# zhyever/Amodal-Depth-Anything

Measured on AMD Instinct MI355X. Metric: images/sec at 518x518 bs=32 ViT-L (AmodalDAv2 forward), higher is better.
Workload: dtype f16

## Files before the change

### amodal-depth-anything_amd/csrc/ada_igemm.hip

```cpp
#include <math.h>
#include <stdarg.h>
#include <stdlib.h>
#include <atomic>
#include <mutex>
#include <type_traits>
#include "ada_common.h"

namespace {


enum { EPI_STD = 0, EPI_GELU = 1, EPI_SHUFFLE = 2, EPI_SWIGLU = 3, EPI_TAIL = 4 };

#ifndef ADA_EPI_NT
#define ADA_EPI_NT 4
#endif
ADA_DEV float4 ld_res4(const float* ptr) {
#if ADA_EPI_NT & 1
    const f32x4 v = __builtin_nontemporal_load((const f32x4*)ptr);
    return make_float4(v[0], v[1], v[2], v[3]);
#else
    return *(const float4*)ptr;
#endif
}
ADA_DEV void st_f32x4(float* ptr, float4 v) {
#if ADA_EPI_NT & 2
    const f32x4 t = {v.x, v.y, v.z, v.w};
    __builtin_nontemporal_store(t, (f32x4*)ptr);
#else
    *(float4*)ptr = v;
#endif
}

struct IgemmDev {
    int M, N, K, a_mode;
// ... 12 lines not shown
    float* out_f32;
    long ldo_f32;
    int map_f32;
    op_t* out_op;
    long ldo_op;
    int map_op;
    int map_h, map_w;
    FastDiv dMapW, dMapHW;
    int shuffle_s, shuffle_c;
    int split_seg;
    int a_dup_seg;
    int split_f8;
    int f8_from, f8_mid;
    unsigned f8_scales;
    int bias_row_mod;
    FastDiv dBiasMod;
    int a_wrap;
    int tap_cols;
    unsigned long long tap_bits[3];
    FastDiv dShC, dShS;
    const float* tail_w;
    float tail_b;
    int tail_act;
    int tiles_m, tiles_n;
    int cps;
    int variant;
    int group_n;
    unsigned long long* dbg;
};

ADA_DEV float gelu_erf(float x) {
    const float a = __builtin_fminf(__builtin_fabsf(x), 12.0f);
    float q = -3.2904290173e-05f;
    q = __builtin_fmaf(q, a, 7.6214928455e-04f);
    q = __builtin_fmaf(q, a, -8.0387993652e-03f);
    q = __builtin_fmaf(q, a, 5.3315321524e-02f);
    q = __builtin_fmaf(q, a, 4.5887145819e-01f);
    q = __builtin_fmaf(q, a, 1.1511568259e+00f);
    q = __builtin_fmaf(q, a, 9.9999958888e-01f);
    const float tail = __builtin_amdgcn_exp2f(-q);
    return __builtin_fmaf(-a, tail, __builtin_fmaxf(x, 0.0f));
}

ADA_DEV void gelu_erf4(float4& v) {
    v.x = gelu_erf(v.x);
    v.y = gelu_erf(v.y);
// ... 477 lines not shown
            if (flags & ADA_EP_BIAS) bias4 = *(const float4*)(p.bias + n);
            tail4 = *(const float4*)(p.tail_w + n);
        }
#pragma unroll
        for (int i = 0; i < TI; ++i) {
            dump(i, 0);
#pragma unroll
            for (int k = 0; k < 32 / RPI; ++k) {
                const int row = k * RPI + rsub;
                const int m = mbase + i * 32 + row;
                const float4 v = *(const float4*)(slab + row * SW + 4 * cg);
                float part = __builtin_fmaxf(v.x + bias4.x, 0.f) * tail4.x + __builtin_fmaxf(v.y + bias4.y, 0.f) * tail4.y +
                             __builtin_fmaxf(v.z + bias4.z, 0.f) * tail4.z + __builtin_fmaxf(v.w + bias4.w, 0.f) * tail4.w;
#pragma unroll
                for (int o = 1; o < CG; o <<= 1) part += __shfl_xor(part, o);
                if (cg == 0 && m < p.M) {
                    float d = part + p.tail_b;
                    if (p.tail_act == ADA_ACT_SIGMOID) d = 1.0f / (1.0f + __expf(-d));
                    else if (p.tail_act == ADA_ACT_RELU) d = __builtin_fmaxf(d, 0.0f);
                    p.out_f32[m] = d;
                }
            }
        }
    } else if (EPI != EPI_SHUFFLE && m0 + BM <= p.M && n0 + BN <= p.N && p.res_row_mod == 0 && p.bias_row_mod == 0 &&
               (!p.out_op || p.map_op == ADA_MAP_PLAIN || (p.map_op == ADA_MAP_PAD && p.map_w >= 8)) &&
               (!p.out_f32 || p.map_f32 == ADA_MAP_PLAIN) &&
               (p.out_f32 || (flags & ADA_EP_RESIDUAL) || (p.ldo_op & 7) == 0)) {
        const bool has_bias = (flags & ADA_EP_BIAS) != 0, has_gamma = (flags & ADA_EP_GAMMA) != 0;
        if (!p.out_f32 && !(flags & ADA_EP_RESIDUAL)) {
            constexpr int CG = GW / 8, RPI = 64 / CG;
            const int rsub = lane / CG, cg = CG == 8 ? ((lane - (rsub >> 1)) & 7) : lane % CG;
            const bool relu = (flags & ADA_EP_RELU_OP) != 0;
            const long ld = p.ldo_op;
#pragma unroll
            for (int g = 0; g < NG; ++g) {
                const int n = nwave + g * GW + 8 * cg;
                float4 b0 = make_float4(0, 0, 0, 0), b1 = b0, g0 = make_float4(1, 1, 1, 1), g1 = g0;
                if (has_bias) { b0 = *(const float4*)(p.bias + n); b1 = *(const float4*)(p.bias + n + 4); }
                if (has_gamma) { g0 = *(const float4*)(p.gamma + n); g1 = *(const float4*)(p.gamma + n + 4); }
                op_t* dst = p.out_op + (long)(mbase + rsub) * ld + n;
                const bool pad = p.map_op == ADA_MAP_PAD;
#pragma unroll
                for (int i = 0; i < TI; ++i) {
                    dump(i, g);
                    PadWalk walk;
                    if (pad) walk = pad_start(p, (uint32_t)(mbase + i * 32 + rsub));
// ... 438 lines not shown
    ADA_REQUIRE(a->out_f32 || a->out_op, ADA_EINVAL, "ada_igemm: no output buffer");
    ADA_REQUIRE((long)a->M < (1L << 24), ADA_EUNSUPPORTED, "ada_igemm: M=%d exceeds 2^24 rows", a->M);
    ADA_REQUIRE(a->a_dup_seg >= 0 && a->a_dup_seg % 64 == 0, ADA_EINVAL, "ada_igemm: a_dup_seg=%d must be a non-negative multiple of 64", a->a_dup_seg);
    if (a->a_dup_seg > 0) {
        const long taps = a->a_mode == ADA_A_CONV3 ? 9 : 1;
        ADA_REQUIRE((long)a->K == 3L * taps * a->a_dup_seg && a->lda >= 2L * a->a_dup_seg, ADA_EINVAL,
                    "ada_igemm: a split A operand needs K == %ld * a_dup_seg and lda >= 2 * a_dup_seg (K=%d a_dup_seg=%d lda=%ld)", 3 * taps, a->K, a->a_dup_seg, (long)a->lda);
    }
    if (a->a_mode == ADA_A_CONV3) {
        ADA_REQUIRE(a->lda % 64 == 0, ADA_EINVAL, "ada_igemm: CONV3 needs lda %% 64 == 0 (got %ld)", (long)a->lda);
        ADA_REQUIRE(a->a_dup_seg > 0 || a->K == 9 * a->lda, ADA_EINVAL, "ada_igemm: CONV3 needs K == 9*lda (K=%d lda=%ld)", a->K, (long)a->lda);
        ADA_REQUIRE(a->Ho > 0 && a->Wo > 0 && (a->stride == 1 || a->stride == 2), ADA_EINVAL, "ada_igemm: bad conv geometry");
        ADA_REQUIRE(a->Hp >= (a->Ho - 1) * a->stride + 3 && a->Wp >= (a->Wo - 1) * a->stride + 3, ADA_EINVAL,
                    "ada_igemm: padded input %dx%d too small for output %dx%d stride %d", a->Hp, a->Wp, a->Ho, a->Wo, a->stride);
        ADA_REQUIRE(a->M % (a->Ho * a->Wo) == 0, ADA_EINVAL, "ada_igemm: M must be batch*Ho*Wo");
    } else {
        ADA_REQUIRE(a->a_mode == ADA_A_PLAIN, ADA_EINVAL, "ada_igemm: unknown a_mode %d", a->a_mode);
        ADA_REQUIRE(a->a_dup_seg > 0 || a->a_wrap > 0 || a->lda >= a->K, ADA_EINVAL, "ada_igemm: lda=%ld < K=%d", (long)a->lda, a->K);
    }
    const int f = a->flags;
    ADA_REQUIRE(!(f & ADA_EP_BIAS) || a->bias, ADA_EINVAL, "ada_igemm: EP_BIAS without bias");
    ADA_REQUIRE(!(f & ADA_EP_GAMMA) || a->gamma, ADA_EINVAL, "ada_igemm: EP_GAMMA without gamma");
    ADA_REQUIRE(!(f & ADA_EP_RESIDUAL) || a->res, ADA_EINVAL, "ada_igemm: EP_RESIDUAL without res");
    const bool tail = (f & ADA_EP_TAIL) != 0, swiglu = (f & ADA_EP_SWIGLU) != 0;
    const bool shuffle = a->out_op && a->map_op == ADA_MAP_SHUFFLE;
    ADA_REQUIRE(a->N % 4 == 0, ADA_EUNSUPPORTED, "ada_igemm: N=%d must be a multiple of 4", a->N);
    ADA_REQUIRE(!a->out_f32 || tail || (a->ldo_f32 % 4 == 0 && ((uintptr_t)a->out_f32 % 16) == 0), ADA_EINVAL, "ada_igemm: out_f32 must be 16-byte aligned with ldo %% 4 == 0");
    ADA_REQUIRE(!a->out_op || (a->ldo_op % 4 == 0 && ((uintptr_t)a->out_op % 8) == 0), ADA_EINVAL, "ada_igemm: out_op must be 8-byte aligned with ldo %% 4 == 0");
    ADA_REQUIRE(!(f & ADA_EP_RESIDUAL) || (a->ldr % 4 == 0 && ((uintptr_t)a->res % 16) == 0), ADA_EINVAL, "ada_igemm: res must be 16-byte aligned with ldr %% 4 == 0");
    ADA_REQUIRE(!(f & ADA_EP_BIAS) || ((uintptr_t)a->bias % 16) == 0, ADA_EINVAL, "ada_igemm: bias must be 16-byte aligned");
    ADA_REQUIRE(!(f & ADA_EP_GAMMA) || ((uintptr_t)a->gamma % 16) == 0, ADA_EINVAL, "ada_igemm: gamma must be 16-byte aligned");
    if (tail) {
        ADA_REQUIRE(a->tail_w && a->out_f32, ADA_EINVAL, "ada_igemm: EP_TAIL needs tail_w and out_f32");
        ADA_REQUIRE(((uintptr_t)a->tail_w % 16) == 0, ADA_EINVAL, "ada_igemm: tail_w must be 16-byte aligned");
        ADA_REQUIRE(a->N <= 64, ADA_EUNSUPPORTED, "ada_igemm: EP_TAIL supports N <= 64 (got %d)", a->N);
        ADA_REQUIRE(!swiglu && !shuffle && !(f & ADA_EP_GELU), ADA_EUNSUPPORTED, "ada_igemm: EP_TAIL cannot be combined with other epilogues");
    }
    if (swiglu) {
        ADA_REQUIRE(a->N % 64 == 0 && a->out_op && !a->out_f32, ADA_EINVAL, "ada_igemm: EP_SWIGLU needs N %% 64 == 0 and only out_op");
        ADA_REQUIRE(a->map_op == ADA_MAP_PLAIN && !(f & (ADA_EP_GELU | ADA_EP_GAMMA | ADA_EP_RESIDUAL)), ADA_EUNSUPPORTED,
                    "ada_igemm: EP_SWIGLU supports bias + MAP_PLAIN only");
    }
    const int maps_needing_grid = (a->out_op && (a->map_op == ADA_MAP_PAD || a->map_op == ADA_MAP_SHUFFLE));
    if (maps_needing_grid) {
        ADA_REQUIRE(a->map_h > 0 && a->map_w > 0 && a->M % (a->map_h * a->map_w) == 0, ADA_EINVAL, "ada_igemm: bad output grid %dx%d for M=%d", a->map_h, a->map_w, a->M);
    }
    if (shuffle) {
        ADA_REQUIRE(a->shuffle_s > 0 && a->shuffle_c > 0 && a->N == a->shuffle_s * a->shuffle_s * a->shuffle_c, ADA_EINVAL,
                    "ada_igemm: SHUFFLE needs N == s*s*c");
        ADA_REQUIRE(a->shuffle_c % 4 == 0 && !a->out_f32 && !(f & ADA_EP_GELU), ADA_EUNSUPPORTED, "ada_igemm: SHUFFLE needs c %% 4 == 0, operand output only");
    }
    const int split_abs = a->split_seg < 0 ? -a->split_seg : a->split_seg;
    if (a->split_seg != 0) {
        ADA_REQUIRE(a->out_op && split_abs % 8 == 0, ADA_EINVAL, "ada_igemm: split_seg needs out_op and a multiple of 8");
        ADA_REQUIRE(a->split_seg > 0 || !shuffle || (a->shuffle_c % 8 == 0 && !(f & ADA_EP_RESIDUAL) && a->ldo_op % 8 == 0), ADA_EUNSUPPORTED,
                    "ada_igemm: the fp8 form of a split output (split_seg < 0) behind MAP_SHUFFLE needs shuffle_c %% 8 == 0, ldo_op %% 8 == 0 and no residual");
        const int cols = shuffle ? a->shuffle_c : swiglu ? a->N / 2 : a->N;
        ADA_REQUIRE(cols <= split_abs && a->ldo_op >= 2L * split_abs, ADA_EINVAL, "ada_igemm: split_seg=%d too small for %d columns / ldo_op=%ld", a->split_seg, cols, (long)a->ldo_op);
    }
    if (a->bias_row_mod != 0) {
        ADA_REQUIRE(a->bias_row_mod > 0 && (f & ADA_EP_BIAS) && a->out_op && !a->out_f32 && !(f & ADA_EP_RESIDUAL) && !tail && !swiglu && !shuffle &&
                    a->ldo_op % 8 == 0 && a->N % 4 == 0, ADA_EUNSUPPORTED,
                    "ada_igemm: bias_row_mod (a bias vector per group of rows) is implemented for operand-typed outputs with ldo_op %% 8 == 0 (bias / GELU epilogues)");
    }
    if (a->a_wrap != 0) {
        ADA_REQUIRE(a->a_mode == ADA_A_PLAIN && a->a_dup_seg == 0 && a->a_wrap > 0 && a->a_wrap % 64 == 0 && a->K == 2 * a->a_wrap && a->lda >= a->a_wrap, ADA_EINVAL,
                    "ada_igemm: a_wrap=%d needs a plain operand, K == 2 * a_wrap (K=%d) and lda >= a_wrap", a->a_wrap, a->K);
    }
    if (a->f8_from != 0) {
        const long per = a->a_mode == ADA_A_CONV3 ? a->lda : (long)a->K;
        ADA_REQUIRE(a->a_dup_seg == 0 && a->a_wrap == 0, ADA_EINVAL, "ada_igemm: f8_from excludes a_dup_seg / a_wrap");
        ADA_REQUIRE(a->f8_from > 0 && a->f8_from % 64 == 0 && a->f8_mid % 64 == 0 && a->f8_from <= a->f8_mid && a->f8_mid <= per && a->f8_from < per, ADA_EINVAL,
                    "ada_igemm: f8_from=%d / f8_mid=%d must be multiples of 64 with 0 < f8_from <= f8_mid <= %ld (the period of the k-walk)", a->f8_from, a->f8_mid, per);
    }
    if (a->tap_cols != 0) {
        ADA_REQUIRE(a->a_mode == ADA_A_CONV3 && a->tap_cols > 0 && a->N % a->tap_cols == 0 && a->N / a->tap_cols <= 16, ADA_EINVAL,
                    "ada_igemm: tap_cols=%d needs a CONV3 operand and N = (1..16) * tap_cols (N=%d)", a->tap_cols, a->N);
        for (int i = 0; i < a->N / a->tap_cols; ++i)
            ADA_REQUIRE(a->tap_mask[i] != 0 && a->tap_mask[i] < 512, ADA_EINVAL, "ada_igemm: tap_mask[%d]=0x%x must name 1..9 of the taps", i, (unsigned)a->tap_mask[i]);
    }
// ... 14 lines not shown
    d.dResMod = make_fastdiv(a->res_row_mod > 0 ? a->res_row_mod : 1);
    d.flags = a->flags;
    d.out_f32 = a->out_f32; d.ldo_f32 = a->ldo_f32; d.map_f32 = a->map_f32;
    d.out_op = (op_t*)a->out_op; d.ldo_op = a->ldo_op; d.map_op = a->map_op;
    d.map_h = a->map_h; d.map_w = a->map_w;
    const bool token = (a->out_f32 && a->map_f32 == ADA_MAP_TOKEN) || (a->out_op && a->map_op == ADA_MAP_TOKEN);
    d.dMapW = make_fastdiv(a->map_w > 0 ? a->map_w : 1);
    d.dMapHW = make_fastdiv(token ? a->map_h : (a->map_h > 0 && a->map_w > 0 ? a->map_h * a->map_w : 1));
    d.shuffle_s = a->shuffle_s; d.shuffle_c = a->shuffle_c;
    d.split_seg = split_abs;
    d.split_f8 = a->split_seg < 0;
    d.f8_from = a->f8_from / 64; d.f8_mid = a->f8_mid / 64; d.f8_scales = a->f8_scales;
    d.a_dup_seg = a->a_dup_seg;
    d.a_wrap = a->a_wrap;
    d.bias_row_mod = a->bias_row_mod;
    d.dBiasMod = make_fastdiv(a->bias_row_mod > 0 ? a->bias_row_mod : 1);
    d.tap_cols = a->tap_cols;
    d.tap_bits[0] = d.tap_bits[1] = d.tap_bits[2] = 0;
    if (a->tap_cols > 0)
        for (int i = 0; i < a->N / a->tap_cols; ++i) d.tap_bits[i / 7] |= (unsigned long long)a->tap_mask[i] << (9 * (i % 7));
    d.dShC = make_fastdiv(a->shuffle_c > 0 ? a->shuffle_c : 1);
    d.dShS = make_fastdiv(a->shuffle_s > 0 ? a->shuffle_s : 1);
    d.tail_w = a->tail_w; d.tail_b = a->tail_b; d.tail_act = a->tail_act;
    d.cps = 0;
    d.group_n = 1;
    d.tiles_m = d.tiles_n = 0;

    apply_env_presets();
    const int force = g_force_tile.load(std::memory_order_relaxed);
    d.dbg = g_dbg.load(std::memory_order_relaxed);
    d.variant = g_variant.load(std::memory_order_relaxed);
    hipStream_t s = (hipStream_t)stream;
    if (tail) return launch_epi<EPI_TAIL>(d, s, a->N <= 32 ? 0 : 1);
    if (swiglu) return launch_epi<EPI_SWIGLU>(d, s, force);
    if (shuffle) return launch_epi<EPI_SHUFFLE>(d, s, force);
    if (f & ADA_EP_GELU) return launch_epi<EPI_GELU>(d, s, force);
    return launch_epi<EPI_STD>(d, s, force);
}
```

### amodal-depth-anything_amd/hip_ext/__init__.py

```python
from __future__ import annotations

import ctypes
import os
from ctypes import c_char_p, c_double, c_float, c_int, c_int32, c_int64, c_uint16, c_void_p
from typing import Optional

import torch

_HERE = os.path.dirname(os.path.abspath(__file__))
_CSRC = os.path.join(os.path.dirname(_HERE), "csrc")

ABI_VERSION = 8
DT_F32, DT_F16, DT_BF16 = 0, 1, 2
A_PLAIN, A_CONV3 = 0, 1
MAP_PLAIN, MAP_PAD, MAP_TOKEN, MAP_SHUFFLE = 0, 1, 2, 3
EP_BIAS, EP_GELU, EP_GAMMA, EP_RESIDUAL, EP_RELU_OP, EP_SWIGLU, EP_TAIL, EP_RELU_F32 = 0x1, 0x2, 0x4, 0x8, 0x10, 0x20, 0x40, 0x80
ACT_NONE, ACT_SIGMOID, ACT_RELU = 0, 1, 2

EXPORTS = (
    "ada_abi_version", "ada_operand_dtype", "ada_last_error", "ada_igemm", "ada_attention_fwd", "ada_attention_ex",
    "ada_pos_embed_resize", "ada_layernorm_fwd", "ada_layernorm_ex", "ada_patchify", "ada_write_cls", "ada_bilinear_fwd", "ada_selftest",
    "ada_minmax_fwd", "ada_depth_stats_fwd", "ada_token_diversity_fwd", "ada_normalize_fwd", "ada_blend_fwd", "ada_depth_eval_fwd", "ada_tile_blend_fwd", "ada_dpt_tail_fwd", "ada_tapsum_resize_fwd",
    "ada_debug_set_tile", "ada_debug_set_variant", "ada_debug_set_group", "ada_debug_last_tile",
    "ada_debug_set_timestamps", "ada_debug_set_attention_variant", "ada_debug_count_saturated",
)

EVAL_N, EVAL_SUM_P, EVAL_SUM_G, EVAL_SUM_PP, EVAL_SUM_PG, EVAL_ABS_REL, EVAL_SQ_REL, EVAL_SQ, EVAL_LOG_SQ, EVAL_LOG, \
    EVAL_LOG10_ABS, EVAL_D1, EVAL_D2, EVAL_D3, EVAL_INV_SQ = range(15)
EVAL_NSUM = 16


class IgemmArgs(ctypes.Structure):
    _fields_ = [
        ("M", c_int32), ("N", c_int32), ("K", c_int32), ("a_mode", c_int32),
        ("A", c_void_p), ("lda", c_int64),
        ("Ho", c_int32), ("Wo", c_int32), ("Hp", c_int32), ("Wp", c_int32), ("stride", c_int32),
        ("W", c_void_p), ("bias", c_void_p), ("gamma", c_void_p), ("res", c_void_p), ("ldr", c_int64),
        ("res_row_mod", c_int32), ("res_row_off", c_int32), ("flags", c_int32),
        ("out_f32", c_void_p), ("ldo_f32", c_int64), ("map_f32", c_int32),
        ("out_op", c_void_p), ("ldo_op", c_int64), ("map_op", c_int32),
        ("map_h", c_int32), ("map_w", c_int32), ("shuffle_s", c_int32), ("shuffle_c", c_int32),
        ("tail_w", c_void_p), ("tail_b", c_float), ("tail_act", c_int32),
        ("split_seg", c_int32), ("a_dup_seg", c_int32),
        ("tap_cols", c_int32), ("tap_mask", c_uint16 * 16), ("a_wrap", c_int32), ("bias_row_mod", c_int32),
        ("f8_from", c_int32), ("f8_mid", c_int32), ("f8_scales", ctypes.c_uint32),
    ]


class LayerNormArgs(ctypes.Structure):
    _fields_ = [
        ("in_", c_void_p), ("ld_in", c_int64), ("rows_out", c_int32), ("dim", c_int32), ("group_in", c_int32), ("skip", c_int32),
        ("weight", c_void_p), ("bias", c_void_p), ("eps", c_float),
        ("out_op", c_void_p), ("ld_op", c_int64), ("map_op", c_int32), ("map_h", c_int32), ("map_w", c_int32), ("relu", c_int32),
        ("out_f32", c_void_p), ("ld_f32", c_int64), ("split_seg", c_int32),
        ("weight2", c_void_p), ("bias2", c_void_p), ("out2_op", c_void_p), ("ld2_op", c_int64),
        ("out2_group", c_int32), ("out2_skip", c_int32), ("split_seg2", c_int32), ("unshuffle_s", c_int32), ("tap_bias", c_void_p), ("identity", c_int32),
    ]


class HipExtError(RuntimeError):
    pass


_lib = None
_lib_path = None


def library_path(bf16: bool = False) -> str:
# ... 119 lines not shown
        ev1.record(torch.cuda.current_stream())
        self.records.setdefault(name, []).append((ev0, ev1, float(work)))

    def summary(self):
        out = {}
        for name, recs in self.records.items():
            ms = sum(a.elapsed_time(b) for a, b, _ in recs)
            out[name] = dict(launches=len(recs), ms_total=ms, ms_avg=ms / len(recs), work_total=sum(w for _, _, w in recs))
        return out


_timer: Optional[KernelTimer] = None


def set_timer(t: Optional[KernelTimer]):
    global _timer
    _timer = t


def igemm(*, M, N, K, A, lda, W, k_alg=None, a_mode=A_PLAIN, conv=None, bias=None, gamma=None, res=None, ldr=0,
          res_row_mod=0, res_row_off=0, flags=0, out_f32=None, ldo_f32=0, map_f32=MAP_PLAIN, out_op=None, ldo_op=0,
          map_op=MAP_PLAIN, map_h=0, map_w=0, shuffle_s=0, shuffle_c=0, tail_w=None, tail_b=0.0, tail_act=ACT_NONE, split_seg=0,
          a_dup_seg=0, tap_cols=0, tap_mask=None, a_wrap=0, bias_row_mod=0,
          f8_from=0, f8_mid=0, f8_scales=0):
    op = operand_dtype()
    a = IgemmArgs()
    a.M, a.N, a.K, a.a_mode = M, N, K, a_mode
    a.A, a.lda = _dev(A, "A", op), lda
    if conv is not None:
        a.Ho, a.Wo, a.Hp, a.Wp, a.stride = conv
    a.W = _dev(W, "W", op)
    a.bias = _opt(bias, "bias", torch.float32)
    a.gamma = _opt(gamma, "gamma", torch.float32)
    a.res, a.ldr = _opt(res, "res", torch.float32), ldr
    a.res_row_mod, a.res_row_off, a.flags = res_row_mod, res_row_off, flags
    a.out_f32, a.ldo_f32, a.map_f32 = _opt(out_f32, "out_f32", torch.float32), ldo_f32, map_f32
    a.out_op, a.ldo_op, a.map_op = _opt(out_op, "out_op", op), ldo_op, map_op
    a.map_h, a.map_w, a.shuffle_s, a.shuffle_c = map_h, map_w, shuffle_s, shuffle_c
    a.tail_w, a.tail_b, a.tail_act = _opt(tail_w, "tail_w", torch.float32), tail_b, tail_act
    a.split_seg = split_seg
    a.a_dup_seg = a_dup_seg
    a.a_wrap = a_wrap
    a.bias_row_mod = bias_row_mod
    a.f8_from, a.f8_mid, a.f8_scales = f8_from, f8_mid, f8_scales
    if tap_cols:
        a.tap_cols = tap_cols
        for i, m in enumerate(tap_mask):
            a.tap_mask[i] = int(m)
    if _timer is not None and _timer.active:
        ev = _timer.start()
        _check(load().ada_igemm(ctypes.byref(a), _stream()), "ada_igemm")
        _timer.stop("igemm", ev, 2.0 * M * N * (k_alg if k_alg is not None else K))
    else:
        _check(load().ada_igemm(ctypes.byref(a), _stream()), "ada_igemm")
    if _tile_log is not None:
        _tile_log.append((M, N, K, load().ada_debug_last_tile()))


def attention(qkv: torch.Tensor, out: torch.Tensor, batch: int, n_tokens: int, heads: int, ld_out: int = 0, split_seg: int = 0):
    op = operand_dtype()
    ev = _timer.start() if (_timer is not None and _timer.active) else None
    if ld_out or split_seg:
        _check(load().ada_attention_ex(_dev(qkv, "qkv", op), _dev(out, "out", op), batch, n_tokens, heads, ld_out, split_seg, _stream()), "ada_attention_ex")
    else:
        _check(load().ada_attention_fwd(_dev(qkv, "qkv", op), _dev(out, "out", op), batch, n_tokens, heads, _stream()),
               "ada_attention_fwd")
    if ev is not None:
# ... 181 lines not shown
```

### amodal-depth-anything_amd/hip_ext/engine.py

```python
from __future__ import annotations

import math
import os
import threading
from collections import OrderedDict
from typing import Dict, Optional

import torch
import torch.nn.functional as F

from . import (A_CONV3, ACT_NONE, ACT_RELU, ACT_SIGMOID, EP_BIAS, EP_GAMMA, EP_GELU, EP_RELU_OP, EP_RESIDUAL,
               EP_SWIGLU, EP_TAIL, MAP_PAD, MAP_SHUFFLE, MAP_TOKEN, HipExtError)
from . import attention as k_attention
from . import bilinear as _bilinear
from . import count_saturated
from . import dpt_tail as k_dpt_tail
from . import igemm as _igemm
from . import layernorm as _layernorm
from . import debug_epoch, instrumented, operand_dtype
from . import depth_stats as k_depth_stats
from . import token_diversity as k_token_diversity
from . import patchify as k_patchify
from . import pos_embed_resize as k_pos_embed_resize
from . import tapsum_resize as k_tapsum_resize
from . import write_cls as k_write_cls

_probe = None


def _probed(kernel, launch):
    def run(*a, **kw):
        launch(*a, **kw)
        t = kw.get("out_op")
        if _probe is not None and t is not None and t.is_contiguous():
            c = torch.zeros(1, dtype=torch.int64, device=t.device)
            count_saturated(t, c)
            _probe.append((f"{kernel} #{len(_probe)} {list(t.shape)}", c))
    return run


k_igemm, k_layernorm, k_bilinear = _probed("igemm", _igemm), _probed("layernorm", _layernorm), _probed("bilinear", _bilinear)

PATCH = 14
LN_EPS = 1e-6
HEAD_GROUPS = ("proj", "projw", "rs0", "rs1", "rs3") + tuple(f"{f}{i}" for f in ("ip", "rn", "rcu", "out") for i in range(4)) + ("oc1", "oc2")
HEAD_ALIASES = {"tok": ("proj", "rs0", "rs1", "rs3"), "ip": tuple(f"ip{i}" for i in range(4)), "rn": tuple(f"rn{i}" for i in range(4)),
                "rcu": tuple(f"rcu{i}" for i in range(4)), "out": tuple(f"out{i}" for i in range(4))}
FUSED_TAIL = os.environ.get("ADA_FUSED_TAIL", "1") == "1"
SUBPIXEL = os.environ.get("ADA_SUBPIXEL", "1") == "1"
SUBPIXEL_SPLIT = os.environ.get("ADA_SUBPIXEL_SPLIT", "1") != "0"
OC1_COMMUTE_SPLIT = os.environ.get("ADA_OC1_COMMUTE_SPLIT", "1") != "0"
STAT_CHUNKS = 8
OC1_COMMUTE = os.environ.get("ADA_OC1_COMMUTE", "1") != "0"


_F8_ENV = os.environ.get("ADA_F8_CORR", "1")
F8_CORR = _F8_ENV != "0"
F8_ENC, F8_HEAD = _F8_ENV in ("1", "enc"), _F8_ENV in ("1", "head")
F8_A_SCALES = 117 | (127 << 16)


def f8_weight_split(wm: torch.Tensor, op, taps: int = 1):
    n = wm.shape[0]
    k = wm.shape[1] // taps
    assert wm.shape[1] == taps * k and k % 128 == 0, (wm.shape, taps)
    w = wm.reshape(n, taps, k).float()
    hi = w.to(op)
    lo = w - hi.float()

    def enc(t):
        m = float(t.abs().max())
        sh = max(-100, min(100, int(math.floor(math.log2(448.0 / m))))) if m > 0 else 0
        q = (t.float() * (2.0 ** sh)).clamp(-448.0, 448.0)
        try:
            b = q.to(torch.float8_e4m3fn).view(torch.uint8)
        except (RuntimeError, TypeError):
# ... 330 lines not shown
            self.o = z(T, wide * D)
            hidden = pw_.blocks[0]["hidden"]
            self.hd = z(T, wide * hidden)
        self.taps = [z(P, m * D) for _ in range(4)]
        G = (D + 63) // 64
        Gi = 0 if head_only else pw_.pe_seg // 64
        self.stat_buf = z(B * (STAT_CHUNKS + G + Gi) * 2, dtype=torch.float32)
        self.stat_sums = self.stat_buf[:B * STAT_CHUNKS * 2].view(B, STAT_CHUNKS, 2)
        self.stat_div = self.stat_buf[B * STAT_CHUNKS * 2:B * (STAT_CHUNKS + G) * 2].view(B, G, 2)
        self.stat_in = self.stat_buf[B * (STAT_CHUNKS + G) * 2:].view(B, Gi, 2) if Gi else None
        if pw_.readout:
            self.cls_op = [z(B, m * D) for _ in range(4)]
            self.cls_bias = [z(B, D, dtype=torch.float32) for _ in range(4)]
            self.taps_ro = [z(P, m * D) for _ in range(4)]
        self.grid = [(4 * ph, 4 * pw), (2 * ph, 2 * pw), (ph, pw), ((ph - 1) // 2 + 1, (pw - 1) // 2 + 1)]
        oc = pw_.oc
        ocp = [_r64(c) for c in oc]
        self.ocp, self.Fp = ocp, Fp
        self.tp = {i: z(B, ph + 2, pw + 2, (2 if pw_.sp[i].get("split") else 1) * ocp[i]) for i in pw_.sp}
        self.t0 = None if 0 in pw_.sp else z(P, mm("rs0") * ocp[0])
        self.t1 = None if 1 in pw_.sp else z(P, mm("rs1") * ocp[1])
        self.pre3 = z(B, ph + 2, pw + 2, mm("rs3") * ocp[3])
        self.L = [None if i in pw_.sp else z(B, g[0] + 2, g[1] + 2, mm(f"{first}{i}") * ocp[i]) for i, g in enumerate(self.grid)]
        if pw_.amodal_head:
            self.ipf = [z(B * g[0] * g[1], oc[i], dtype=torch.float32) for i, g in enumerate(self.grid)]
            self.L2 = [z(B, g[0] + 2, g[1] + 2, mm(f"rn{i}") * ocp[i]) for i, g in enumerate(self.grid)]
        self.rnx = [z(B * g[0] * g[1], Fch, dtype=torch.float32) for g in self.grid]
        self.spf = {} if pw_.amodal_head else {i: z(B * self.grid[i][0] * self.grid[i][1], Fch, dtype=torch.float32) for i in pw_.sp}
        self.rnr = [z(B, g[0] + 2, g[1] + 2, mm(f"rcu{i}") * Fp) for i, g in enumerate(self.grid)]
        self.tmpa = [z(B, g[0] + 2, g[1] + 2, mm(f"rcu{i}") * Fp) for i, g in enumerate(self.grid)]
        rows = [B * g[0] * g[1] for g in self.grid]
        lvl0 = z(2 * rows[0] * Fch, dtype=torch.float32)
        self.r = [lvl0[:rows[0] * Fch].view(rows[0], Fch)]
        self.s = [lvl0[rows[0] * Fch:].view(rows[0], Fch)]
        for i in range(1, 4):
            if pw_.amodal_head and oc[i] >= Fch:
                self.r.append(self.ipf[i].view(-1)[:rows[i] * Fch].view(rows[i], Fch))
            else:
                self.r.append(z(rows[i], Fch, dtype=torch.float32))
            self.s.append(z(rows[i], Fch, dtype=torch.float32))
        self.sr = [z(B, g[0] + 2, g[1] + 2, mm(f"rcu{i}") * Fp) for i, g in enumerate(self.grid)]
        self.u = [z(B * g[0] * g[1], mm(f"out{i}") * Fp) for i, g in enumerate(self.grid)]
        self.zf = self.rnx
        g0 = self.grid[0]
        self.g296 = (2 * g0[0], 2 * g0[1])
        self.p1 = None if pw_.oc1c is not None else z(B, self.g296[0] + 2, self.g296[1] + 2, mm("oc1") * Fp)
        self.tmaps = z(rows[0], 9 * (Fch // 2)) if pw_.oc1c is not None else None
        half = Fch // 2
        self.half, self.halfp = half, _r64(half)
        self.oc1 = lvl0.view(B * self.g296[0] * self.g296[1], half)
        self.fused_tail = FUSED_TAIL and fused_tail_applies(half, self.halfp, self.g296[0], H, pw_.split)
        self.fin = None if self.fused_tail else z(B, H + 2, W + 2, mm("oc2") * self.halfp)


LADDER_GUARD = float(os.environ.get("ADA_LADDER_GUARD", "0.02"))
LADDER_STICKY = os.environ.get("ADA_LADDER_STICKY", "1") != "0"
HEAD_STREAMS = os.environ.get("ADA_HEAD_STREAMS", "auto")
HEAD_STREAMS_ROWS = int(os.environ.get("ADA_HEAD_STREAMS_ROWS", str(12 * 1369)))
GRAPH_MODE = os.environ.get("ADA_GRAPH", "auto")
# ... 613 lines not shown
                s_ = 4 if i == 0 else 2
                if i in w.sp:
                    k_igemm(M=P, N=oc[i], k_alg=D, A=taps_in[i], W=w.proj_w[i], **self._kdup(KD, w.proj_w[i], a_seg=ws.tap_seg), bias=w.proj_b[i], flags=EP_BIAS,
                            out_op=ws.tp[i], ldo_op=ws.tp[i].shape[3], map_op=MAP_PAD, map_h=ph, map_w=pw, split_seg=-ocp[i] if w.sp[i].get("split") else 0)
                    return
                t = ws.t0 if i == 0 else ws.t1
                rs_w, rs_b = (w.rs0_w, w.rs0_b) if i == 0 else (w.rs1_w, w.rs1_b)
                k_igemm(M=P, N=oc[i], k_alg=D, A=taps_in[i], W=w.proj_w[i], **self._kdup(KD, w.proj_w[i], a_seg=ws.tap_seg), bias=w.proj_b[i], flags=EP_BIAS, out_op=t, ldo_op=t.shape[1], split_seg=S(f"rs{i}", ocp[i]))
                k_igemm(M=P, N=s_ * s_ * oc[i], k_alg=oc[i], A=t, W=rs_w, bias=rs_b, flags=EP_BIAS, **self._kdup(t.shape[1], rs_w),
                        out_op=ws.L[i], ldo_op=ws.L[i].shape[3], map_op=MAP_SHUFFLE, map_h=ph, map_w=pw, shuffle_s=s_, shuffle_c=oc[i], split_seg=S(f"{first}{i}", ocp[i]))
            elif i == 2:
                k_igemm(M=P, N=oc[2], k_alg=D, A=taps_in[2], W=w.proj_w[2], **self._kdup(KD, w.proj_w[2], a_seg=ws.tap_seg), bias=w.proj_b[2], flags=EP_BIAS,
                        out_op=ws.L[2], ldo_op=ws.L[2].shape[3], map_op=MAP_PAD, map_h=ph, map_w=pw, split_seg=S(first + "2", ocp[2]))
            else:
                k_igemm(M=P, N=oc[3], k_alg=D, A=taps_in[3], W=w.proj_w[3], **self._kdup(KD, w.proj_w[3], a_seg=ws.tap_seg), bias=w.proj_b[3], flags=EP_BIAS,
                        out_op=ws.pre3, ldo_op=ws.pre3.shape[3], map_op=MAP_PAD, map_h=ph, map_w=pw, split_seg=S("rs3", ocp[3]))
                self._conv3(ws.pre3, w.rs3_w, rows[3], oc[3], grid[3], stride=2, cin=oc[3], bias=w.rs3_b, flags=EP_BIAS,
                            out_op=ws.L[3], ldo_op=ws.L[3].shape[3], map_op=MAP_PAD, map_h=grid[3][0], map_w=grid[3][1], split_seg=S(first + "3", ocp[3]))

        def input_projection(i):
            if i in w.sp:
                sp = w.sp[i]
                ncol = sp["s"] * sp["s"] * oc[i]
                self._conv3(ws.tp[i], sp["w"], P, ncol, (ph, pw), k_alg=sp["taps_per_col"] * oc[i], bias=sp["b"], flags=EP_BIAS,
                            out_f32=ws.ipf[i], ldo_f32=ncol, tap_cols=oc[i], tap_mask=sp["masks"])
                k_layernorm(ws.ipf[i], ncol, rows[i], oc[i], w.ip_ln_w[i], w.ip_ln_b[i], LN_EPS, out_op=ws.L2[i], ld_op=ws.L2[i].shape[3],
                            map_op=MAP_PAD, map_h=grid[i][0], map_w=grid[i][1], relu=True, split_seg=S(f"rn{i}", ocp[i]),
                            unshuffle_s=sp["s"], tap_bias=sp["tapb"])
                return
            self._conv3(ws.L[i], w.ip_w[i], rows[i], oc[i], grid[i], cin=oc[i], bias=w.ip_b[i], flags=EP_BIAS, out_f32=ws.ipf[i], ldo_f32=oc[i])
            k_layernorm(ws.ipf[i], oc[i], rows[i], oc[i], w.ip_ln_w[i], w.ip_ln_b[i], LN_EPS, out_op=ws.L2[i],
                        ld_op=ws.L2[i].shape[3], map_op=MAP_PAD, map_h=grid[i][0], map_w=grid[i][1], relu=True, split_seg=S(f"rn{i}", ocp[i]))

        def layer_rn(i):
            if not w.amodal_head and i in w.sp:
                sp = w.sp[i]
                ncol = sp["s"] * sp["s"] * Fch
                self._conv3(ws.tp[i], sp["w"], P, ncol, (ph, pw), k_alg=sp["taps_per_col"] * oc[i], bias=sp["b"], flags=EP_BIAS,
                            out_f32=ws.spf[i], ldo_f32=ncol, tap_cols=Fch, tap_mask=sp["masks"])
                k_layernorm(ws.spf[i], ncol, rows[i], Fch, None, None, LN_EPS, identity=True, relu=2, out_f32=ws.rnx[i], ld_f32=Fch, out_op=ws.rnr[i],
                            ld_op=ws.rnr[i].shape[3], map_op=MAP_PAD, map_h=grid[i][0], map_w=grid[i][1], split_seg=S(f"rcu{i}", Fp),
                            unshuffle_s=sp["s"], tap_bias=sp["tapb"])
                return
            src = ws.L2[i] if w.amodal_head else ws.L[i]
            self._conv3(src, w.rn_w[i], rows[i], Fch, grid[i], cin=oc[i], flags=EP_RELU_OP, out_f32=ws.rnx[i], ldo_f32=Fch,
                        out_op=ws.rnr[i], ldo_op=ws.rnr[i].shape[3], map_op=MAP_PAD, map_h=grid[i][0], map_w=grid[i][1], split_seg=S(f"rcu{i}", Fp))
# ... 66 lines not shown
```

### include/ada_hip.h

```cpp
#ifndef ADA_HIP_H
#define ADA_HIP_H

#include <stdint.h>

#ifdef __cplusplus
extern "C" {
#endif

#define ADA_ABI_VERSION 8

#define ADA_OK 0
#define ADA_EINVAL (-1)
#define ADA_EUNSUPPORTED (-2)
#define ADA_ELAUNCH (-3)

#define ADA_DT_F32 0
#define ADA_DT_F16 1
#define ADA_DT_BF16 2

int ada_abi_version(void);
int ada_operand_dtype(void);
const char* ada_last_error(void);


#define ADA_A_PLAIN 0
#define ADA_A_CONV3 1

#define ADA_MAP_PLAIN 0
#define ADA_MAP_PAD 1
#define ADA_MAP_TOKEN 2
#define ADA_MAP_SHUFFLE 3

#define ADA_EP_BIAS 0x1
#define ADA_EP_GELU 0x2
#define ADA_EP_GAMMA 0x4
#define ADA_EP_RESIDUAL 0x8
#define ADA_EP_RELU_OP 0x10
#define ADA_EP_SWIGLU 0x20
#define ADA_EP_TAIL 0x40
#define ADA_EP_RELU_F32 0x80

#define ADA_ACT_NONE 0
#define ADA_ACT_SIGMOID 1
#define ADA_ACT_RELU 2

typedef struct ada_igemm_args {
    int32_t M, N, K;
    int32_t a_mode;
    const void* A;
    int64_t lda;
    int32_t Ho, Wo, Hp, Wp, stride;
    const void* W;
    const float* bias;
    const float* gamma;
    const float* res;
    int64_t ldr;
    int32_t res_row_mod;
    int32_t res_row_off;
    int32_t flags;
    float* out_f32;
    int64_t ldo_f32;
    int32_t map_f32;
    void* out_op;
    int64_t ldo_op;
    int32_t map_op;
    int32_t map_h, map_w;
    int32_t shuffle_s;
    int32_t shuffle_c;
    const float* tail_w;
    float tail_b;
    int32_t tail_act;
    int32_t split_seg;
    int32_t a_dup_seg;
    int32_t tap_cols;
    uint16_t tap_mask[16];
    int32_t a_wrap;
    int32_t bias_row_mod;
    int32_t f8_from, f8_mid;
    uint32_t f8_scales;
} ada_igemm_args;

int ada_igemm(const ada_igemm_args* args, void* stream);

int ada_attention_fwd(const void* qkv, void* out, int32_t batch, int32_t n_tokens, int32_t heads,
                      void* stream);
int ada_attention_ex(const void* qkv, void* out, int32_t batch, int32_t n_tokens, int32_t heads, int64_t ld_out, int32_t split_seg,
                     void* stream);

int ada_layernorm_fwd(const float* in, int64_t ld_in, int32_t rows_out, int32_t dim,
                      int32_t group_in, int32_t skip,
                      const float* weight, const float* bias, float eps,
                      void* out_op, int64_t ld_op, int32_t map_op, int32_t map_h, int32_t map_w,
                      int32_t relu,
                      float* out_f32, int64_t ld_f32, int32_t split_seg, void* stream);

typedef struct ada_layernorm_args {
    const float* in;
    int64_t ld_in;
    int32_t rows_out, dim, group_in, skip;
    const float* weight;
    const float* bias;
    float eps;
// ... 87 lines not shown
```

Baseline: 622.9.

## Fuse channel LayerNorm and ReLU into sub-pixel conv GEMM epilogue

Adds an EPI_CHANLN epilogue to the implicit-GEMM kernel that applies bias, corrects border taps, computes a per-pixel LayerNorm over the 256 channels of each tile with cross-wave shared-memory reductions, applies ReLU, and writes the padded operand-typed output at sub-pixel positions. The amodal head's 256-channel sub-pixel convolutions use it in place of writing an fp32 intermediate and running a separate LayerNorm kernel. This removes one fp32 round trip through memory and a kernel launch per level. In exchange the tile is pinned to 256x256, each tile gains two extra block-wide syncs, and border handling adds branching.

Result: no change. 627.3, median of 6 (+0.7%).

```diff
diff --git a/amodal-depth-anything_amd/csrc/ada_igemm.hip b/amodal-depth-anything_amd/csrc/ada_igemm.hip
--- a/amodal-depth-anything_amd/csrc/ada_igemm.hip
+++ b/amodal-depth-anything_amd/csrc/ada_igemm.hip
@@ -9,7 +9,7 @@
 namespace {
 
 
-enum { EPI_STD = 0, EPI_GELU = 1, EPI_SHUFFLE = 2, EPI_SWIGLU = 3, EPI_TAIL = 4 };
+enum { EPI_STD = 0, EPI_GELU = 1, EPI_SHUFFLE = 2, EPI_SWIGLU = 3, EPI_TAIL = 4, EPI_CHANLN = 5 };
 
 #ifndef ADA_EPI_NT
 #define ADA_EPI_NT 4
@@ -68,6 +68,11 @@
     const float* tail_w;
     float tail_b;
     int tail_act;
+    const float* ln_gamma;
+    const float* ln_beta;
+    float ln_eps;
+    const float* tap_bias;
+    int ln_s;
     int tiles_m, tiles_n;
     int cps;
     int variant;
@@ -591,6 +596,98 @@
                 }
             }
         }
+    } else if constexpr (EPI == EPI_CHANLN) {
+        static_assert(BN == 256 && NG == 1 && GW == 64 && WAVES_N == 4, "the channel LayerNorm epilogue is built for the 256 x 256 tile, 4 waves across");
+        constexpr int CG = GW / 8, RPI = 64 / CG, NKI = 32 / RPI;
+        float* red_sum = (float*)(smem + NWAVES * 32 * SW * 4);
+        float* red_sq = red_sum + BM * WAVES_N;
+        static_assert(NWAVES * 32 * SW * 4 + 2 * BM * WAVES_N * 4 <= 2 * STAGE_BYTES, "LayerNorm partials must fit behind the epilogue slabs");
+        const int rsub = lane / CG, cg = (lane - (rsub >> 1)) & 7;
+        const int n = nwave + 8 * cg;
+        const int c = n - n0;
+        const int phase = n0 / BN;
+        const int ss = p.ln_s, py = phase / ss, px = phase - py * ss;
+        const int fh = p.map_h, fw = p.map_w;
+        const float4 b0 = *(const float4*)(p.bias + n), b1 = *(const float4*)(p.bias + n + 4);
+        const float4 g0 = *(const float4*)(p.ln_gamma + c), g1 = *(const float4*)(p.ln_gamma + c + 4);
+        const float4 e0 = *(const float4*)(p.ln_beta + c), e1 = *(const float4*)(p.ln_beta + c + 4);
+        const bool relu = (flags & ADA_EP_RELU_OP) != 0;
+        const long ld = p.ldo_op;
+#pragma unroll
+        for (int i = 0; i < TI; ++i) {
+            dump(i, 0);
+            const int rbase = wm * TI * 32 + i * 32 + rsub;
+            float4 v[NKI][2];
+            long orow[NKI];
+#pragma unroll
+            for (int k = 0; k < NKI; ++k) {
+                const int row = k * RPI + rsub;
+                const int m = mbase + i * 32 + row;
+                float4 x0 = *(const float4*)(slab + row * SW + 8 * cg);
+                float4 x1 = *(const float4*)(slab + row * SW + 8 * cg + 4);
+                x0.x += b0.x; x0.y += b0.y; x0.z += b0.z; x0.w += b0.w;
+                x1.x += b1.x; x1.y += b1.y; x1.z += b1.z; x1.w += b1.w;
+                uint32_t b, rem, cy, cx;
+                fast_divmod((uint32_t)(m < p.M ? m : -1 + p.M), p.dHoWo, b, rem);
+                fast_divmod(rem, p.dWo, cy, cx);
+                const int Y = (int)cy * ss + py, X = (int)cx * ss + px;
+                orow[k] = m < p.M ? ((long)b * (fh + 2) + (Y + 1)) * (fw + 2) + (X + 1) : -1;
+                if (p.tap_bias) {
+                    unsigned ring = 0;
+                    if (Y == 0) ring |= 0x007u;
+                    if (Y == fh - 1) ring |= 0x1c0u;
+                    if (X == 0) ring |= 0x049u;
+                    if (X == fw - 1) ring |= 0x124u;
+                    if (ring) {
+                        const float* tb = p.tap_bias + (long)n * 9;
+                        for (int t = 0; t < 9; ++t)
+                            if ((ring >> t) & 1u) {
+                                x0.x -= tb[t]; x0.y -= tb[9 + t]; x0.z -= tb[18 + t]; x0.w -= tb[27 + t];
+                                x1.x -= tb[36 + t]; x1.y -= tb[45 + t]; x1.z -= tb[54 + t]; x1.w -= tb[63 + t];
+                            }
+                    }
+                }
+                v[k][0] = x0;
+                v[k][1] = x1;
+                float sm = ((x0.x + x0.y) + (x0.z + x0.w)) + ((x1.x + x1.y) + (x1.z + x1.w));
+                sm += __shfl_xor(sm, 1);
+                sm += __shfl_xor(sm, 2);
+                sm += __shfl_xor(sm, 4);
+                if ((lane & 7) == 0) red_sum[(rbase + k * RPI) * WAVES_N + wn] = sm;
+            }
+            __syncthreads();
+            float mean[NKI];
+#pragma unroll
+            for (int k = 0; k < NKI; ++k) {
+                const float4 t = *(const float4*)(red_sum + (rbase + k * RPI) * WAVES_N);
+                mean[k] = ((t.x + t.y) + (t.z + t.w)) / (float)BN;
+                const float4 x0 = v[k][0], x1 = v[k][1];
+                const float a0 = x0.x - mean[k], a1 = x0.y - mean[k], a2 = x0.z - mean[k], a3 = x0.w - mean[k];
+                const float a4 = x1.x - mean[k], a5 = x1.y - mean[k], a6 = x1.z - mean[k], a7 = x1.w - mean[k];
+                float q = ((a0 * a0 + a1 * a1) + (a2 * a2 + a3 * a3)) + ((a4 * a4 + a5 * a5) + (a6 * a6 + a7 * a7));
+                q += __shfl_xor(q, 1);
+                q += __shfl_xor(q, 2);
+                q += __shfl_xor(q, 4);
+                if ((lane & 7) == 0) red_sq[(rbase + k * RPI) * WAVES_N + wn] = q;
+            }
+            __syncthreads();
+#pragma unroll
+            for (int k = 0; k < NKI; ++k) {
+                const float4 t = *(const float4*)(red_sq + (rbase + k * RPI) * WAVES_N);
+                const float rstd = 1.0f / sqrtf(((t.x + t.y) + (t.z + t.w)) / (float)BN + p.ln_eps);
+                const float mu = mean[k];
+                float4 y0, y1;
+                y0.x = (v[k][0].x - mu) * rstd * g0.x + e0.x; y0.y = (v[k][0].y - mu) * rstd * g0.y + e0.y;
+                y0.z = (v[k][0].z - mu) * rstd * g0.z + e0.z; y0.w = (v[k][0].w - mu) * rstd * g0.w + e0.w;
+                y1.x = (v[k][1].x - mu) * rstd * g1.x + e1.x; y1.y = (v[k][1].y - mu) * rstd * g1.y + e1.y;
+                y1.z = (v[k][1].z - mu) * rstd * g1.z + e1.z; y1.w = (v[k][1].w - mu) * rstd * g1.w + e1.w;
+                if (relu) {
+                    y0.x = __builtin_fmaxf(y0.x, 0.f); y0.y = __builtin_fmaxf(y0.y, 0.f); y0.z = __builtin_fmaxf(y0.z, 0.f); y0.w = __builtin_fmaxf(y0.w, 0.f);
+                    y1.x = __builtin_fmaxf(y1.x, 0.f); y1.y = __builtin_fmaxf(y1.y, 0.f); y1.z = __builtin_fmaxf(y1.z, 0.f); y1.w = __builtin_fmaxf(y1.w, 0.f);
+                }
+                if (orow[k] >= 0) store_op8(p, p.out_op + orow[k] * ld + c, c, y0, y1);
+            }
+        }
     } else if (EPI != EPI_SHUFFLE && m0 + BM <= p.M && n0 + BN <= p.N && p.res_row_mod == 0 && p.bias_row_mod == 0 &&
                (!p.out_op || p.map_op == ADA_MAP_PLAIN || (p.map_op == ADA_MAP_PAD && p.map_w >= 8)) &&
                (!p.out_f32 || p.map_f32 == ADA_MAP_PLAIN) &&
@@ -1075,8 +1172,23 @@
     ADA_REQUIRE(!(f & ADA_EP_BIAS) || a->bias, ADA_EINVAL, "ada_igemm: EP_BIAS without bias");
     ADA_REQUIRE(!(f & ADA_EP_GAMMA) || a->gamma, ADA_EINVAL, "ada_igemm: EP_GAMMA without gamma");
     ADA_REQUIRE(!(f & ADA_EP_RESIDUAL) || a->res, ADA_EINVAL, "ada_igemm: EP_RESIDUAL without res");
-    const bool tail = (f & ADA_EP_TAIL) != 0, swiglu = (f & ADA_EP_SWIGLU) != 0;
+    const bool tail = (f & ADA_EP_TAIL) != 0, swiglu = (f & ADA_EP_SWIGLU) != 0, chanln = (f & ADA_EP_CHANLN) != 0;
     const bool shuffle = a->out_op && a->map_op == ADA_MAP_SHUFFLE;
+    int ln_s = 0;
+    if (chanln) {
+        ADA_REQUIRE(a->a_mode == ADA_A_CONV3 && a->stride == 1 && a->tap_cols == 256 && (f & ADA_EP_BIAS) && a->ln_gamma && a->ln_beta, ADA_EINVAL,
+                    "ada_igemm: EP_CHANLN needs a stride-1 CONV3 sub-pixel convolution with tap_cols == 256 (got %d), EP_BIAS, ln_gamma and ln_beta", a->tap_cols);
+        ADA_REQUIRE(a->out_op && !a->out_f32 && a->map_op == ADA_MAP_PAD && a->bias_row_mod == 0 &&
+                    !(f & (ADA_EP_GELU | ADA_EP_GAMMA | ADA_EP_RESIDUAL | ADA_EP_SWIGLU | ADA_EP_TAIL | ADA_EP_RELU_F32)), ADA_EUNSUPPORTED,
+                    "ada_igemm: EP_CHANLN writes one operand-typed MAP_PAD output (bias, optional ReLU; no fp32 output, residual, GELU, LayerScale)");
+        ln_s = a->map_h / a->Ho;
+        ADA_REQUIRE(ln_s >= 1 && a->map_h == ln_s * a->Ho && a->map_w == ln_s * a->Wo && a->N == ln_s * ln_s * a->tap_cols, ADA_EINVAL,
+                    "ada_igemm: EP_CHANLN needs the fine grid map_h x map_w = s * (Ho x Wo) and N = s * s * 256 (map %dx%d, conv %dx%d, N=%d)", a->map_h, a->map_w, a->Ho, a->Wo, a->N);
+        ADA_REQUIRE(a->ldo_op % 8 == 0 && ((uintptr_t)a->out_op % 16) == 0 && ((uintptr_t)a->ln_gamma % 16) == 0 && ((uintptr_t)a->ln_beta % 16) == 0, ADA_EINVAL,
+                    "ada_igemm: EP_CHANLN needs out_op 16-byte aligned with ldo_op %% 8 == 0 and 16-byte aligned ln_gamma / ln_beta");
+    } else {
+        ADA_REQUIRE(!a->tap_bias, ADA_EINVAL, "ada_igemm: tap_bias without EP_CHANLN");
+    }
     ADA_REQUIRE(a->N % 4 == 0, ADA_EUNSUPPORTED, "ada_igemm: N=%d must be a multiple of 4", a->N);
     ADA_REQUIRE(!a->out_f32 || tail || (a->ldo_f32 % 4 == 0 && ((uintptr_t)a->out_f32 % 16) == 0), ADA_EINVAL, "ada_igemm: out_f32 must be 16-byte aligned with ldo %% 4 == 0");
     ADA_REQUIRE(!a->out_op || (a->ldo_op % 4 == 0 && ((uintptr_t)a->out_op % 8) == 0), ADA_EINVAL, "ada_igemm: out_op must be 8-byte aligned with ldo %% 4 == 0");
@@ -1094,7 +1206,7 @@
         ADA_REQUIRE(a->map_op == ADA_MAP_PLAIN && !(f & (ADA_EP_GELU | ADA_EP_GAMMA | ADA_EP_RESIDUAL)), ADA_EUNSUPPORTED,
                     "ada_igemm: EP_SWIGLU supports bias + MAP_PLAIN only");
     }
-    const int maps_needing_grid = (a->out_op && (a->map_op == ADA_MAP_PAD || a->map_op == ADA_MAP_SHUFFLE));
+    const int maps_needing_grid = (a->out_op && (a->map_op == ADA_MAP_PAD || a->map_op == ADA_MAP_SHUFFLE)) && !chanln;
     if (maps_needing_grid) {
         ADA_REQUIRE(a->map_h > 0 && a->map_w > 0 && a->M % (a->map_h * a->map_w) == 0, ADA_EINVAL, "ada_igemm: bad output grid %dx%d for M=%d", a->map_h, a->map_w, a->M);
     }
@@ -1108,7 +1220,7 @@
         ADA_REQUIRE(a->out_op && split_abs % 8 == 0, ADA_EINVAL, "ada_igemm: split_seg needs out_op and a multiple of 8");
         ADA_REQUIRE(a->split_seg > 0 || !shuffle || (a->shuffle_c % 8 == 0 && !(f & ADA_EP_RESIDUAL) && a->ldo_op % 8 == 0), ADA_EUNSUPPORTED,
                     "ada_igemm: the fp8 form of a split output (split_seg < 0) behind MAP_SHUFFLE needs shuffle_c %% 8 == 0, ldo_op %% 8 == 0 and no residual");
-        const int cols = shuffle ? a->shuffle_c : swiglu ? a->N / 2 : a->N;
+        const int cols = shuffle ? a->shuffle_c : swiglu ? a->N / 2 : chanln ? a->tap_cols : a->N;
         ADA_REQUIRE(cols <= split_abs && a->ldo_op >= 2L * split_abs, ADA_EINVAL, "ada_igemm: split_seg=%d too small for %d columns / ldo_op=%ld", a->split_seg, cols, (long)a->ldo_op);
     }
     if (a->bias_row_mod != 0) {
@@ -1169,6 +1281,7 @@
     d.dShC = make_fastdiv(a->shuffle_c > 0 ? a->shuffle_c : 1);
     d.dShS = make_fastdiv(a->shuffle_s > 0 ? a->shuffle_s : 1);
     d.tail_w = a->tail_w; d.tail_b = a->tail_b; d.tail_act = a->tail_act;
+    d.ln_gamma = a->ln_gamma; d.ln_beta = a->ln_beta; d.ln_eps = a->ln_eps; d.tap_bias = a->tap_bias; d.ln_s = ln_s;
     d.cps = 0;
     d.group_n = 1;
     d.tiles_m = d.tiles_n = 0;
@@ -1178,6 +1291,7 @@
     d.dbg = g_dbg.load(std::memory_order_relaxed);
     d.variant = g_variant.load(std::memory_order_relaxed);
     hipStream_t s = (hipStream_t)stream;
+    if (chanln) return launch_cfg<256, 256, 64, 2, 4, EPI_CHANLN>(d, s);
     if (tail) return launch_epi<EPI_TAIL>(d, s, a->N <= 32 ? 0 : 1);
     if (swiglu) return launch_epi<EPI_SWIGLU>(d, s, force);
     if (shuffle) return launch_epi<EPI_SHUFFLE>(d, s, force);
diff --git a/amodal-depth-anything_amd/hip_ext/__init__.py b/amodal-depth-anything_amd/hip_ext/__init__.py
--- a/amodal-depth-anything_amd/hip_ext/__init__.py
+++ b/amodal-depth-anything_amd/hip_ext/__init__.py
@@ -10,11 +10,12 @@
 _HERE = os.path.dirname(os.path.abspath(__file__))
 _CSRC = os.path.join(os.path.dirname(_HERE), "csrc")
 
-ABI_VERSION = 8
+ABI_VERSION = 9
 DT_F32, DT_F16, DT_BF16 = 0, 1, 2
 A_PLAIN, A_CONV3 = 0, 1
 MAP_PLAIN, MAP_PAD, MAP_TOKEN, MAP_SHUFFLE = 0, 1, 2, 3
 EP_BIAS, EP_GELU, EP_GAMMA, EP_RESIDUAL, EP_RELU_OP, EP_SWIGLU, EP_TAIL, EP_RELU_F32 = 0x1, 0x2, 0x4, 0x8, 0x10, 0x20, 0x40, 0x80
+EP_CHANLN = 0x400
 ACT_NONE, ACT_SIGMOID, ACT_RELU = 0, 1, 2
 
 EXPORTS = (
@@ -44,6 +45,7 @@
         ("split_seg", c_int32), ("a_dup_seg", c_int32),
         ("tap_cols", c_int32), ("tap_mask", c_uint16 * 16), ("a_wrap", c_int32), ("bias_row_mod", c_int32),
         ("f8_from", c_int32), ("f8_mid", c_int32), ("f8_scales", ctypes.c_uint32),
+        ("ln_gamma", c_void_p), ("ln_beta", c_void_p), ("ln_eps", c_float), ("tap_bias", c_void_p),
     ]
 
 
@@ -209,7 +211,7 @@
           res_row_mod=0, res_row_off=0, flags=0, out_f32=None, ldo_f32=0, map_f32=MAP_PLAIN, out_op=None, ldo_op=0,
           map_op=MAP_PLAIN, map_h=0, map_w=0, shuffle_s=0, shuffle_c=0, tail_w=None, tail_b=0.0, tail_act=ACT_NONE, split_seg=0,
           a_dup_seg=0, tap_cols=0, tap_mask=None, a_wrap=0, bias_row_mod=0,
-          f8_from=0, f8_mid=0, f8_scales=0):
+          f8_from=0, f8_mid=0, f8_scales=0, ln_gamma=None, ln_beta=None, ln_eps=0.0, tap_bias=None):
     op = operand_dtype()
     a = IgemmArgs()
     a.M, a.N, a.K, a.a_mode = M, N, K, a_mode
@@ -230,6 +232,8 @@
     a.a_wrap = a_wrap
     a.bias_row_mod = bias_row_mod
     a.f8_from, a.f8_mid, a.f8_scales = f8_from, f8_mid, f8_scales
+    a.ln_gamma, a.ln_beta, a.ln_eps = _opt(ln_gamma, "ln_gamma", torch.float32), _opt(ln_beta, "ln_beta", torch.float32), ln_eps
+    a.tap_bias = _opt(tap_bias, "tap_bias", torch.float32)
     if tap_cols:
         a.tap_cols = tap_cols
         for i, m in enumerate(tap_mask):
diff --git a/amodal-depth-anything_amd/hip_ext/engine.py b/amodal-depth-anything_amd/hip_ext/engine.py
--- a/amodal-depth-anything_amd/hip_ext/engine.py
+++ b/amodal-depth-anything_amd/hip_ext/engine.py
@@ -9,7 +9,7 @@
 import torch
 import torch.nn.functional as F
 
-from . import (A_CONV3, ACT_NONE, ACT_RELU, ACT_SIGMOID, EP_BIAS, EP_GAMMA, EP_GELU, EP_RELU_OP, EP_RESIDUAL,
+from . import (A_CONV3, ACT_NONE, ACT_RELU, ACT_SIGMOID, EP_BIAS, EP_CHANLN, EP_GAMMA, EP_GELU, EP_RELU_OP, EP_RESIDUAL,
                EP_SWIGLU, EP_TAIL, MAP_PAD, MAP_SHUFFLE, MAP_TOKEN, HipExtError)
 from . import attention as k_attention
 from . import bilinear as _bilinear
@@ -52,6 +52,7 @@
 OC1_COMMUTE_SPLIT = os.environ.get("ADA_OC1_COMMUTE_SPLIT", "1") != "0"
 STAT_CHUNKS = 8
 OC1_COMMUTE = os.environ.get("ADA_OC1_COMMUTE", "1") != "0"
+HEAD_EPI = os.environ.get("ADA_HEAD_EPI", "1") != "0"
 
 
 _F8_ENV = os.environ.get("ADA_F8_CORR", "1")
@@ -428,8 +429,9 @@
         self.t1 = None if 1 in pw_.sp else z(P, mm("rs1") * ocp[1])
         self.pre3 = z(B, ph + 2, pw + 2, mm("rs3") * ocp[3])
         self.L = [None if i in pw_.sp else z(B, g[0] + 2, g[1] + 2, mm(f"{first}{i}") * ocp[i]) for i, g in enumerate(self.grid)]
+        self.chanln = {i for i in pw_.sp if pw_.amodal_head and oc[i] == 256} if HEAD_EPI else set()
         if pw_.amodal_head:
-            self.ipf = [z(B * g[0] * g[1], oc[i], dtype=torch.float32) for i, g in enumerate(self.grid)]
+            self.ipf = [None if i in self.chanln else z(B * g[0] * g[1], oc[i], dtype=torch.float32) for i, g in enumerate(self.grid)]
             self.L2 = [z(B, g[0] + 2, g[1] + 2, mm(f"rn{i}") * ocp[i]) for i, g in enumerate(self.grid)]
         self.rnx = [z(B * g[0] * g[1], Fch, dtype=torch.float32) for g in self.grid]
         self.spf = {} if pw_.amodal_head else {i: z(B * self.grid[i][0] * self.grid[i][1], Fch, dtype=torch.float32) for i in pw_.sp}
@@ -440,7 +442,7 @@
         self.r = [lvl0[:rows[0] * Fch].view(rows[0], Fch)]
         self.s = [lvl0[rows[0] * Fch:].view(rows[0], Fch)]
         for i in range(1, 4):
-            if pw_.amodal_head and oc[i] >= Fch:
+            if pw_.amodal_head and oc[i] >= Fch and self.ipf[i] is not None:
                 self.r.append(self.ipf[i].view(-1)[:rows[i] * Fch].view(rows[i], Fch))
             else:
                 self.r.append(z(rows[i], Fch, dtype=torch.float32))
@@ -1100,6 +1102,11 @@
             if i in w.sp:
                 sp = w.sp[i]
                 ncol = sp["s"] * sp["s"] * oc[i]
+                if i in ws.chanln:
+                    self._conv3(ws.tp[i], sp["w"], P, ncol, (ph, pw), k_alg=sp["taps_per_col"] * oc[i], bias=sp["b"], flags=EP_BIAS | EP_CHANLN | EP_RELU_OP,
+                                tap_cols=oc[i], tap_mask=sp["masks"], ln_gamma=w.ip_ln_w[i], ln_beta=w.ip_ln_b[i], ln_eps=LN_EPS, tap_bias=sp["tapb"],
+                                out_op=ws.L2[i], ldo_op=ws.L2[i].shape[3], map_op=MAP_PAD, map_h=grid[i][0], map_w=grid[i][1], split_seg=S(f"rn{i}", ocp[i]))
+                    return
                 self._conv3(ws.tp[i], sp["w"], P, ncol, (ph, pw), k_alg=sp["taps_per_col"] * oc[i], bias=sp["b"], flags=EP_BIAS,
                             out_f32=ws.ipf[i], ldo_f32=ncol, tap_cols=oc[i], tap_mask=sp["masks"])
                 k_layernorm(ws.ipf[i], ncol, rows[i], oc[i], w.ip_ln_w[i], w.ip_ln_b[i], LN_EPS, out_op=ws.L2[i], ld_op=ws.L2[i].shape[3],
diff --git a/include/ada_hip.h b/include/ada_hip.h
--- a/include/ada_hip.h
+++ b/include/ada_hip.h
@@ -7,7 +7,7 @@
 extern "C" {
 #endif
 
-#define ADA_ABI_VERSION 8
+#define ADA_ABI_VERSION 9
 
 #define ADA_OK 0
 #define ADA_EINVAL (-1)
@@ -39,6 +39,7 @@
 #define ADA_EP_SWIGLU 0x20
 #define ADA_EP_TAIL 0x40
 #define ADA_EP_RELU_F32 0x80
+#define ADA_EP_CHANLN 0x400
 
 #define ADA_ACT_NONE 0
 #define ADA_ACT_SIGMOID 1
@@ -78,6 +79,10 @@
     int32_t bias_row_mod;
     int32_t f8_from, f8_mid;
     uint32_t f8_scales;
+    const float* ln_gamma;
+    const float* ln_beta;
+    float ln_eps;
+    const float* tap_bias;
 } ada_igemm_args;
 
 int ada_igemm(const ada_igemm_args* args, void* stream);
```
